# jstrom2002/ImageCodecs

Measured on NVIDIA B200. Metric: jpeg_encode_mp_per_s, higher is better.
Workload: dtype f32

## Files before the change

### imagecodecs_b200/csrc/jpeg_tables.h

```cpp
#pragma once
#include <stddef.h>
#include <stdint.h>

namespace jg {

#define JG_ZZ_INIT                                                                              \
    { 0, 1, 5, 6, 14, 15, 27, 28, 2, 4, 7, 13, 16, 26, 29, 42, 3, 8, 12, 17, 25, 30, 41, 43,    \
      9, 11, 18, 24, 31, 40, 44, 53, 10, 19, 23, 32, 39, 45, 52, 54, 20, 22, 33, 38, 46, 51,    \
      55, 60, 21, 34, 37, 47, 50, 56, 59, 61, 35, 36, 48, 49, 57, 58, 62, 63 }

enum HuffTable { HT_LUMA_DC = 0, HT_LUMA_AC = 1, HT_CHROMA_DC = 2, HT_CHROMA_AC = 3 };

enum Layout { LAYOUT_444 = 0, LAYOUT_420 = 1, LAYOUT_GRAY = 2 };

struct QuantSet {
    float luma[64];
    float chroma[64];
};

struct HuffLut {
    uint32_t ac[2][256];
    uint32_t dc[2][16];
};

bool build_qt(int quality_mode, int quality, uint8_t qt_luma[64], uint8_t qt_chroma[64]);
void build_pqt(const uint8_t qt[64], float pqt[64]);
void build_huff_lut(HuffLut* lut);
size_t emit_headers(int w, int h, int ncomp_out, int subsampling, const uint8_t qt_luma[64],
                    const uint8_t qt_chroma[64], uint8_t* out, size_t cap, int restart_interval = 0);
size_t schedule_words(int n_images);
size_t build_schedule(const int* tiles_per_image, int n_images, uint32_t* out);

}
```

### imagecodecs_b200/csrc/jpeg_transform.cuh

```cuda
#pragma once
#include "jpeg_kernel.cuh"

namespace jg {

template <int LAYOUT>
struct TGeo {
    static constexpr int BPM = LAYOUT == LAYOUT_444 ? 3 : (LAYOUT == LAYOUT_420 ? 6 : 1);
    static constexpr int ITER_MCUS = LAYOUT == LAYOUT_420 ? 2 : 8;
    static constexpr int ITERS = LAYOUT == LAYOUT_444 ? 4 : 8;
    static constexpr int ITEM_MCUS = ITER_MCUS * ITERS;
    static constexpr int ITER_BLOCKS = ITER_MCUS * BPM;
    static constexpr int GROUP_FLOATS = LAYOUT == LAYOUT_444 ? 3 * 2 * kTileFloats : (LAYOUT == LAYOUT_420 ? 6 * kTileFloats : 2 * kTileFloats);
    static constexpr int GROUPS = LAYOUT == LAYOUT_420 ? 2 : 4;
    static constexpr int MCU_PAD = LAYOUT == LAYOUT_420 ? 48 : (LAYOUT == LAYOUT_444 ? 24 : 0);
    static constexpr int STAGE_INT16 = ITER_BLOCKS * kCoefStride + ITER_MCUS * MCU_PAD;
    static JG_DEV int stage_off(int b) { return b * kCoefStride + (b / BPM) * MCU_PAD; }
    static JG_DEV int stage_off(int mcu, int j) { return (mcu * BPM + j) * kCoefStride + mcu * MCU_PAD; }
};
static_assert(TGeo<LAYOUT_444>::ITEM_MCUS == transform_item_mcus(LAYOUT_444) && TGeo<LAYOUT_420>::ITEM_MCUS == transform_item_mcus(LAYOUT_420) &&
              TGeo<LAYOUT_GRAY>::ITEM_MCUS == transform_item_mcus(LAYOUT_GRAY), "host and kernel agree on the item size");

template <int LAYOUT>
struct TWarp {
    using G = TGeo<LAYOUT>;
    alignas(16) float xch[G::GROUPS * G::GROUP_FLOATS];
    alignas(16) int16_t stage[G::STAGE_INT16];
};
template <int LAYOUT>
struct TSmem { TWarp<LAYOUT> wm[kWarps]; };

struct TLane {
    float pq_l[8], pq_c[8];
    unsigned zz2[8];
};

constexpr float kFloorMagic = 12582912.0f - 1024.0f;
JG_DEV void quantise2(f32x2 c, float pq, unsigned& kx, unsigned& ky)
{
    const f32x2 b = f2_add(f2_add(f2_mul(c, f2(pq, pq)), f2(1024.0f, 1024.0f)), f2(0.5f, 0.5f));
    const f32x2 r = f2_add_rd(b, f2(kFloorMagic, kFloorMagic));
    kx = f_bits(r.x);
    ky = f_bits(r.y);
}
JG_DEV unsigned quantise1(float c, float pq)
{
    return f_bits(f_add_rd(f_add(f_add(f_mul(c, pq), 1024.0f), 0.5f), kFloorMagic));
}
template <int NC>
JG_DEV void rgb_biased(const uint32_t* w, int i, float& r, float& g, float& b)
{
    if (NC == 4) { r = u8_biased(w[i], 0); g = u8_biased(w[i], 1); b = u8_biased(w[i], 2); }
    else {
        r = u8_biased(w[(3 * i) >> 2], (3 * i) & 3);
        g = u8_biased(w[(3 * i + 1) >> 2], (3 * i + 1) & 3);
        b = u8_biased(w[(3 * i + 2) >> 2], (3 * i + 2) & 3);
    }
}
#ifndef JG_U8_VIA_PRMT
#define JG_U8_VIA_PRMT 1
#endif
template <int NC>
JG_DEV void rgb_pair(const uint32_t* wa, const uint32_t* wb, int ia, int ib, f32x2& R, f32x2& G, f32x2& B)
{
    float r0, g0, b0, r1, g1, b1;
#if JG_U8_VIA_PRMT
    rgb_biased<NC>(wa, ia, r0, g0, b0);
    rgb_biased<NC>(wb, ib, r1, g1, b1);
    const f32x2 bias = f2(kU8Bias, kU8Bias);
    R = f2_sub(f2(r0, r1), bias); G = f2_sub(f2(g0, g1), bias); B = f2_sub(f2(b0, b1), bias);
#else
    rgb_of<NC>(wa, ia, r0, g0, b0);
    rgb_of<NC>(wb, ib, r1, g1, b1);
    R = f2(r0, r1); G = f2(g0, g1); B = f2(b0, b1);
#endif
}

struct TAddr {
    unsigned xch;
    unsigned stage;
};

template <int LAYOUT>
JG_DEV void stage_to_global(unsigned stage, int16_t* gout, int nblk)
{
    using G = TGeo<LAYOUT>;
    const int t = JG_TID & 31;
#pragma unroll
    for (int q = 0; q < (G::ITER_BLOCKS * 8 + 31) / 32; ++q) {
        const int c = q * 32 + t, blk = c >> 3, part = c & 7;
        if (blk < nblk) *reinterpret_cast<uint4*>(gout + blk * 64 + part * 8) = lds_v4(stage + (unsigned)(G::stage_off(blk) + part * 8) * 2u);
    }
}

template <int LAYOUT, int NC>
struct TPixels {
    static constexpr int WORDS = LAYOUT == LAYOUT_420 ? 16 * NC / 4 : (LAYOUT == LAYOUT_444 ? 8 * NC / 4 : 2);
    uint32_t a[WORDS];
    uint32_t b[LAYOUT == LAYOUT_420 ? 1 : WORDS];
};

template <int LAYOUT, int NC>
JG_DEV void fetch_pixels(const ImageDesc& im, int my0, int mx0, int nM, TPixels<LAYOUT, NC>& px)
{
    const int t = JG_TID & 31, u = t & 7;
#pragma unroll
    for (int i = 0; i < TPixels<LAYOUT, NC>::WORDS; ++i) px.a[i] = 0u;
    if (LAYOUT == LAYOUT_420) {
        const int grp = t >> 4, r16 = t & 15;
        if (grp < nM) {
            int my, mx;
            mcu_pos(im, my0, mx0, grp, my, mx);
            int y = my * 16 + r16; if (y >= im.h) y = im.h - 1;
            load_segment<NC, 16>(im, mx * 16, y, reinterpret_cast<uint32_t (&)[16 * NC / 4]>(px.a));
        }
    } else {
        constexpr int C = LAYOUT == LAYOUT_444 ? NC : 1;
        const int g = t >> 3;
        const int sa = LAYOUT == LAYOUT_444 ? g : 2 * g, sb = LAYOUT == LAYOUT_444 ? g + 4 : 2 * g + 1;
#pragma unroll
        for (int i = 0; i < TPixels<LAYOUT, NC>::WORDS; ++i) px.b[i] = 0u;
        if (sa < nM) {
            int my, mx;
            mcu_pos(im, my0, mx0, sa, my, mx);
            int y = my * 8 + u; if (y >= im.h) y = im.h - 1;
            load_segment<C, 8>(im, mx * 8, y, reinterpret_cast<uint32_t (&)[8 * C / 4]>(px.a));
        }
        if (sb < nM) {
            int my, mx;
            mcu_pos(im, my0, mx0, sb, my, mx);
            int y = my * 8 + u; if (y >= im.h) y = im.h - 1;
            load_segment<C, 8>(im, mx * 8, y, reinterpret_cast<uint32_t (&)[8 * C / 4]>(px.b));
        }
    }
}

template <int NC, class Prefetch>
JG_DEV void transform_iter_444(const TAddr& A, const TPixels<LAYOUT_444, NC>& px, int nM, int16_t* gout, const TLane& LC, Prefetch&& prefetch)
{
    const int t = JG_TID & 31, u = t & 7, g = t >> 3;
    f32x2 sy[8], sb[8], sr[8];
#pragma unroll
    for (int i = 0; i < 8; ++i) {
        f32x2 R, Gc, B;
        rgb_pair<NC>(px.a, px.b, i, i, R, Gc, B);
        sy[i] = f2_sub(f2_add(f2_add(f2_mul(f2(0.299f, 0.299f), R), f2_mul(f2(0.587f, 0.587f), Gc)), f2_mul(f2(0.114f, 0.114f), B)),
                       f2(128.0f, 128.0f));
        sb[i] = f2_add(f2_sub(f2_mul(f2(-0.1687f, -0.1687f), R), f2_mul(f2(0.3313f, 0.3313f), Gc)), f2_mul(f2(0.5f, 0.5f), B));
        sr[i] = f2_sub(f2_sub(f2_mul(f2(0.5f, 0.5f), R), f2_mul(f2(0.4187f, 0.4187f), Gc)), f2_mul(f2(0.0813f, 0.0813f), B));
    }
    prefetch();
    const unsigned row = A.xch + (unsigned)(u * 9) * 8u;
    aan8x2(sy);
#pragma unroll
    for (int i = 0; i < 8; ++i) sts_v2f(row + 8u * i, sy[i]);
    aan8x2(sb);
#pragma unroll
    for (int i = 0; i < 8; ++i) sts_v2f(row + 8u * (kTileFloats + i), sb[i]);
    aan8x2(sr);
#pragma unroll
    for (int i = 0; i < 8; ++i) sts_v2f(row + 8u * (2 * kTileFloats + i), sr[i]);
    warp_sync();
    const unsigned colA = A.xch + 8u * (unsigned)u;
#pragma unroll
    for (int c = 0; c < 3; ++c) {
        f32x2 col[8];
#pragma unroll
        for (int v = 0; v < 8; ++v) col[v] = lds_v2f(colA + 8u * (unsigned)(c * kTileFloats + v * 9));
        aan8x2(col);
        const unsigned dA = A.stage + 2u * (unsigned)TGeo<LAYOUT_444>::stage_off(g, c), dB = A.stage + 2u * (unsigned)TGeo<LAYOUT_444>::stage_off(g + 4, c);
#pragma unroll
        for (int v = 0; v < 8; ++v) {
            unsigned ka, kb;
            quantise2(col[v], c ? LC.pq_c[v] : LC.pq_l[v], ka, kb);
            sts_u16(dA + LC.zz2[v], ka);
            sts_u16(dB + LC.zz2[v], kb);
        }
    }
    warp_sync();
    stage_to_global<LAYOUT_444>(A.stage, gout, nM * 3);
}

template <int NC, class Prefetch>
JG_DEV void transform_iter_420(const TAddr& A, const TPixels<LAYOUT_420, NC>& px, int nM, int16_t* gout, const TLane& LC, Prefetch&& prefetch)
{
    const int t = JG_TID & 31, u = t & 7, grp = t >> 4, r16 = t & 15, h = r16 >> 3;
    const unsigned ypair = A.xch;
    const unsigned ctile = A.xch + 4u * (4 * kTileFloats);
    const bool valid = grp < nM;
    f32x2 cbs[4], crs[4];
    f32x2 sy[8];
#pragma unroll
    for (int j = 0; j < 4; ++j) {
        f32x2 cb[2], cr[2];
#pragma unroll
        for (int e = 0; e < 2; ++e) {
            const int i = 2 * j + e;
            f32x2 R, Gc, B;
            rgb_pair<NC>(px.a, px.a, i, i + 8, R, Gc, B);
            sy[i] = f2_sub(f2_add(f2_add(f2_mul(f2(0.299f, 0.299f), R), f2_mul(f2(0.587f, 0.587f), Gc)),
                                  f2_mul(f2(0.114f, 0.114f), B)), f2(128.0f, 128.0f));
            cb[e] = f2_add(f2_sub(f2_mul(f2(-0.1687f, -0.1687f), R), f2_mul(f2(0.3313f, 0.3313f), Gc)),
                           f2_mul(f2(0.5f, 0.5f), B));
            cr[e] = f2_sub(f2_sub(f2_mul(f2(0.5f, 0.5f), R), f2_mul(f2(0.4187f, 0.4187f), Gc)),
                           f2_mul(f2(0.0813f, 0.0813f), B));
        }
        cbs[j] = f2_add(cb[0], cb[1]);
        crs[j] = f2_add(cr[0], cr[1]);
    }
    prefetch();
    aan8x2(sy);
    if (valid) {
        const unsigned ty = ypair + 8u * (unsigned)(h * kTileFloats + (r16 & 7) * 9);
#pragma unroll
        for (int i = 0; i < 8; ++i) sts_v2f(ty + 8u * i, sy[i]);
    }
    const bool even = (r16 & 1) == 0;
    float samp[8];
#pragma unroll
    for (int i = 0; i < 4; ++i) {
        const f32x2 mine = even ? cbs[i] : crs[i], give = even ? crs[i] : cbs[i];
        const f32x2 other = f2(warp_shfl_xor_f32(give.x, 1), warp_shfl_xor_f32(give.y, 1));
        const f32x2 q = f2_mul(f2_add(mine, other), f2(0.25f, 0.25f));
        samp[i] = q.x; samp[4 + i] = q.y;
    }
    aan8(samp);
    if (valid) {
        const unsigned tc = ctile + 4u * (unsigned)((r16 & 1) * kTileFloats + (r16 >> 1) * 9);
#pragma unroll
        for (int i = 0; i < 8; ++i) sts_f32(tc + 4u * i, samp[i]);
    }
    warp_sync();
    if (valid) {
        f32x2 col[8];
#pragma unroll
        for (int v = 0; v < 8; ++v) col[v] = lds_v2f(ypair + 8u * (unsigned)(h * kTileFloats + v * 9 + u));
        aan8x2(col);
        const unsigned dL = A.stage + 2u * (unsigned)TGeo<LAYOUT_420>::stage_off(grp, 2 * h), dR = dL + 2u * kCoefStride;
#pragma unroll
        for (int v = 0; v < 8; ++v) {
            unsigned kl, kr;
            quantise2(col[v], LC.pq_l[v], kl, kr);
            sts_u16(dL + LC.zz2[v], kl);
            sts_u16(dR + LC.zz2[v], kr);
        }
        float c[8];
#pragma unroll
        for (int v = 0; v < 8; ++v) c[v] = lds_f32(ctile + 4u * (unsigned)(h * kTileFloats + v * 9 + u));
        aan8(c);
        const unsigned dC = A.stage + 2u * (unsigned)TGeo<LAYOUT_420>::stage_off(grp, 4 + h);
#pragma unroll
        for (int v = 0; v < 8; ++v) sts_u16(dC + LC.zz2[v], quantise1(c[v], LC.pq_c[v]));
    }
    warp_sync();
    stage_to_global<LAYOUT_420>(A.stage, gout, nM * 6);
}

template <class Prefetch>
JG_DEV void transform_iter_gray(const TAddr& A, const TPixels<LAYOUT_GRAY, 1>& px, int nM, int16_t* gout, const TLane& LC, Prefetch&& prefetch)
{
    const int t = JG_TID & 31, u = t & 7, g = t >> 3;
    f32x2 s[8];
#if JG_U8_VIA_PRMT
#pragma unroll
    for (int i = 0; i < 8; ++i)
        s[i] = f2_sub(f2_sub(f2(u8_biased(px.a[i >> 2], i & 3), u8_biased(px.b[i >> 2], i & 3)), f2(kU8Bias, kU8Bias)), f2(128.0f, 128.0f));
#else
#pragma unroll
    for (int i = 0; i < 8; ++i) s[i] = f2_sub(f2(u8_to_f(byte_of(px.a, i)), u8_to_f(byte_of(px.b, i))), f2(128.0f, 128.0f));
#endif
    prefetch();
    aan8x2(s);
#pragma unroll
    for (int i = 0; i < 8; ++i) sts_v2f(A.xch + 8u * (unsigned)(u * 9 + i), s[i]);
    warp_sync();
    f32x2 col[8];
#pragma unroll
    for (int v = 0; v < 8; ++v) col[v] = lds_v2f(A.xch + 8u * (unsigned)(v * 9 + u));
    aan8x2(col);
    const unsigned dA = A.stage + 2u * (unsigned)((2 * g) * kCoefStride), dB = dA + 2u * kCoefStride;
#pragma unroll
    for (int v = 0; v < 8; ++v) {
        unsigned ka, kb;
        quantise2(col[v], LC.pq_l[v], ka, kb);
        sts_u16(dA + LC.zz2[v], ka);
        sts_u16(dB + LC.zz2[v], kb);
    }
    warp_sync();
    stage_to_global<LAYOUT_GRAY>(A.stage, gout, nM);
}

#ifndef JG_TR_MINB
#define JG_TR_MINB (LAYOUT == LAYOUT_444 ? 3 : 4)
#endif
template <int LAYOUT, int NC>
JG_KERNEL(kThreads, JG_TR_MINB)
void transform_kernel(const JG_GRID_CONSTANT TransformParams P, const JG_GRID_CONSTANT QuantSet Q)
{
    using G = TGeo<LAYOUT>;
    JG_DYNAMIC_SMEM(smem_raw);
    TSmem<LAYOUT>& S = *reinterpret_cast<TSmem<LAYOUT>*>(smem_raw);
    const int t = JG_TID;
    const unsigned item = (unsigned)JG_CTA_ID * (unsigned)kWarps + (unsigned)(t >> 5);
    if (item >= (unsigned)P.n_items) return;
    TLane LC;
    {
        const int u = t & 7;
#pragma unroll
        for (int v = 0; v < 8; ++v) {
            LC.pq_l[v] = Q.luma[8 * v + u];
            LC.pq_c[v] = Q.chroma[8 * v + u];
            LC.zz2[v] = 2u * (unsigned)zz_of(8 * v + u);
        }
    }
    unsigned img, local;
    if (P.items_per_image > 0) {
        img = item / (unsigned)P.items_per_image;
        local = item - img * (unsigned)P.items_per_image;
    } else {
        unsigned lo = 0, hi = (unsigned)P.n_images - 1u;
        while (lo < hi) {
            const unsigned mid = (lo + hi + 1u) >> 1;
            if (ldg_u32(P.first_item + mid) <= item) lo = mid; else hi = mid - 1u;
        }
        img = lo;
        local = item - ldg_u32(P.first_item + lo);
    }
    const ImageDesc im = P.images[img];
    TWarp<LAYOUT>& W = S.wm[t >> 5];
    TAddr A;
    A.xch = smem_addr(W.xch) + 4u * (unsigned)(((t & 31) / (32 / G::GROUPS)) * G::GROUP_FLOATS);
    A.stage = smem_addr(W.stage);
    const int m_begin = (int)local * G::ITEM_MCUS;
    const int m_end = (im.n_mcus - m_begin < G::ITEM_MCUS) ? im.n_mcus : m_begin + G::ITEM_MCUS;
    int16_t* gout = P.coefs + (im.first_block + (unsigned long long)m_begin * G::BPM) * 64ull;
    int my0 = m_begin / im.mcus_x, mx0 = m_begin - my0 * im.mcus_x;
    TPixels<LAYOUT, NC> px;
    fetch_pixels<LAYOUT, NC>(im, my0, mx0, m_end - m_begin < G::ITER_MCUS ? m_end - m_begin : G::ITER_MCUS, px);
#pragma unroll 1
    for (int m0 = m_begin; m0 < m_end; m0 += G::ITER_MCUS) {
        const int nM = m_end - m0 < G::ITER_MCUS ? m_end - m0 : G::ITER_MCUS;
        int mx1 = mx0 + G::ITER_MCUS, my1 = my0;
        while (mx1 >= im.mcus_x) { mx1 -= im.mcus_x; ++my1; }
        const int left = m_end - m0 - G::ITER_MCUS;
        const int nM1 = left < 0 ? 0 : (left < G::ITER_MCUS ? left : G::ITER_MCUS);
        TPixels<LAYOUT, NC> nx;
        auto prefetch = [&]() { fetch_pixels<LAYOUT, NC>(im, my1, mx1, nM1, nx); };
        if constexpr (LAYOUT == LAYOUT_444) transform_iter_444<NC>(A, px, nM, gout, LC, prefetch);
        else if constexpr (LAYOUT == LAYOUT_420) transform_iter_420<NC>(A, px, nM, gout, LC, prefetch);
        else transform_iter_gray(A, px, nM, gout, LC, prefetch);
        px = nx;
        gout += G::ITER_BLOCKS * 64;
        mx0 = mx1; my0 = my1;
    }
}

}
```

### imagecodecs_b200/csrc/jpeg_device.h

```cpp
#pragma once
#include <stdint.h>

#if defined(JG_EMULATE)
#include "cuda_emu.h"
#else
#include <cuda_runtime.h>

#define JG_DEV __device__ __forceinline__
#define JG_DEV_NOINLINE __device__ __noinline__
#define JG_TID ((int)threadIdx.x)
#define JG_CTA_ID ((int)blockIdx.x)
#define JG_GRID_DIM ((int)gridDim.x)
#define JG_KERNEL(threads, min_ctas) __global__ __launch_bounds__(threads, min_ctas)
#define JG_GRID_CONSTANT __grid_constant__
#define JG_DYNAMIC_SMEM(name) extern __shared__ __align__(16) unsigned char name[]
#define JG_CONST_TABLE static __device__ __constant__
#define JG_WARP_ANY(x) __any_sync(0xffffffffu, (x))
#define JG_RECONVERGE() __syncwarp()

namespace jg {

JG_DEV float f_add(float a, float b) { return __fadd_rn(a, b); }
JG_DEV float f_sub(float a, float b) { return __fsub_rn(a, b); }
JG_DEV float f_mul(float a, float b) { return __fmul_rn(a, b); }
// ... 95 lines not shown
JG_DEV void mbar_init(unsigned long long* bar, unsigned arrivals)
{
    asm volatile("mbarrier.init.shared::cta.b64 [%0], %1;" ::"r"(smem_addr(bar)), "r"(arrivals) : "memory");
}
JG_DEV void mbar_fence_init() { asm volatile("fence.mbarrier_init.release.cluster;" ::: "memory"); }
JG_DEV void mbar_expect_tx(unsigned long long* bar, unsigned bytes)
{
    asm volatile("mbarrier.arrive.expect_tx.shared::cta.b64 _, [%0], %1;" ::"r"(smem_addr(bar)), "r"(bytes) : "memory");
}
JG_DEV void bulk_g2s(void* dst_smem, const void* src_gmem, unsigned bytes, unsigned long long* bar)
{
    asm volatile("cp.async.bulk.shared::cluster.global.mbarrier::complete_tx::bytes [%0], [%1], %2, [%3];"
                 ::"r"(smem_addr(dst_smem)), "l"(src_gmem), "r"(bytes), "r"(smem_addr(bar)) : "memory");
}
JG_DEV void fence_proxy_async() { asm volatile("fence.proxy.async.shared::cta;" ::: "memory"); }
JG_DEV void tma_load_2d(void* dst_smem, const void* tmap, int c0, int c1, unsigned long long* bar)
{
    asm volatile("cp.async.bulk.tensor.2d.shared::cluster.global.tile.mbarrier::complete_tx::bytes [%0], [%1, {%2, %3}], [%4];"
                 ::"r"(smem_addr(dst_smem)), "l"(tmap), "r"(c0), "r"(c1), "r"(smem_addr(bar)) : "memory");
}
JG_DEV void mbar_wait(unsigned long long* bar, unsigned parity)
{
    asm volatile(
        "{\n"
        ".reg .pred p;\n"
        "WAIT_%=:\n"
        "mbarrier.try_wait.parity.shared::cta.b64 p, [%0], %1;\n"
        "@!p bra WAIT_%=;\n"
        "}\n" ::"r"(smem_addr(bar)), "r"(parity) : "memory");
}

}
#endif
```

### imagecodecs_b200/csrc/jpeg_entropy.cu

```cuda
#include "jpeg_entropy.cuh"
#include "jpeg_launch.h"

namespace jg {

template <int MODE>
static cudaError_t entropy_prepare_mode(int* ctas)
{
    auto kern = entropy_kernel<MODE>;
    const int smem = (int)sizeof(EntSmem);
    cudaError_t e = cudaFuncSetAttribute(kern, cudaFuncAttributeMaxDynamicSharedMemorySize, smem);
    if (e != cudaSuccess) return e;
    int n = 0;
    e = cudaOccupancyMaxActiveBlocksPerMultiprocessor(&n, kern, kEntThreads, smem);
    if (n < *ctas) *ctas = n;
    return e;
}

cudaError_t entropy_prepare(int* ctas_per_sm)
{
    int ctas = 1 << 20;
    cudaError_t e = entropy_prepare_mode<kEntModePlain>(&ctas);
    if (e == cudaSuccess) e = entropy_prepare_mode<kEntModeRestart>(&ctas);
    *ctas_per_sm = ctas;
    return e;
}

cudaError_t entropy_launch(int grid, cudaStream_t stream, const LaunchParams& P, const CoefMap& cmap, bool restart)
{
    const size_t smem = sizeof(EntSmem);
    if (restart) entropy_kernel<kEntModeRestart><<<grid, kEntThreads, smem, stream>>>(P, cmap);
    else entropy_kernel<kEntModePlain><<<grid, kEntThreads, smem, stream>>>(P, cmap);
    return cudaGetLastError();
}

}
```

### imagecodecs_b200/csrc/jpeg_entropy.cuh

```cuda
#pragma once
#include "jpeg_kernel.cuh"

namespace jg {

constexpr int kEntBlocks = 32;
constexpr int kEntCoefStride = 72;
#ifndef JG_ENT_SUBWORDS
#define JG_ENT_SUBWORDS 24
#endif
constexpr int kSubWords = JG_ENT_SUBWORDS;
constexpr int kEntRegionWords = 768;
#ifndef JG_ENT_PIECE
#define JG_ENT_PIECE 96
#endif
constexpr int kOnePieceSymbols = JG_ENT_PIECE * kSubWords;
constexpr int kSlowBlocks = 4;
constexpr int kEntModePlain = 0, kEntModeRestart = 2;
constexpr unsigned kEntStageBytes = kEntBlocks * kEntCoefStride * 2;
constexpr unsigned kTabRunBytes = 136u, kTabAcBytes = 16u * kTabRunBytes;
constexpr unsigned kTabDc = 0u, kTabAc = 2u, kTabChroma = 1u, kTabAcChroma = kTabAcBytes / 128u;
static_assert(kTabAcBytes % 128u == 0u, "table offsets are multiples of 128 bytes");

struct EntWarp {
    alignas(128) int16_t coef[kEntBlocks * kEntCoefStride];
// ... 333 lines not shown
        flush_region(W.region, tg, pd.last && hi == nblk, reinterpret_cast<uint8_t*>(pd.raw), pd.raw_cap, k, hb, pos, cap_overflow);
    }
    if (lane == 0) {
        if (pd.last) P.raw_bytes[pd.img_idx] = pos;
        if (cap_overflow) gmem_atomic_or(P.img_status + pd.img_idx, 1u);
    }
    warp_sync();
    clear_region(W.region, kEntRegionWords + 8);
    return true;
}

template <int MODE>
JG_KERNEL(kEntThreads, JG_ENT_MINB)
void entropy_kernel(const JG_GRID_CONSTANT LaunchParams P, const JG_GRID_CONSTANT CoefMap cmap)
{
    constexpr bool restart = MODE == kEntModeRestart;
    JG_DYNAMIC_SMEM(smem_raw);
    EntSmem& S = *reinterpret_cast<EntSmem*>(smem_raw);
    const int t = JG_TID, lane = t & 31;
    for (int i = t; i < 32 + 512; i += kEntThreads) {
        const int cls = i < 32 ? i >> 4 : (i - 32) >> 8, k = i < 32 ? i & 15 : (i - 32) & 255;
        const unsigned h = i < 32 ? P.huff->dc[cls][k] : P.huff->ac[cls][k];
        uint2 e;
        e.x = h >> 8;
        e.y = (h & 0xffu) + (unsigned)(k & 15);
        S.tab.e[i < 32 ? i : (256u + (unsigned)cls * kTabAcBytes) / 8u + (unsigned)(k >> 4) * 17u + (unsigned)(k & 15)] = e;
    }
    EntWarp& W = S.wm[t >> 5];
    const EntTables& T = S.tab;
    if (lane == 0) mbar_init(&W.mbar, 1u);
    clear_region(W.region, kEntRegionWords + 8);
    if (lane < 4) { uint2 z; z.x = 0u; z.y = 0u; W.rec[kEntBlocks + lane] = z; }
    mbar_fence_init();
    cta_sync();

    const int bpm = P.bpm, bpt = P.blocks_per_tile;
    const int lane_j = lane % bpm;
    unsigned phase = 0;
    PendingOut po;
    for (int slot = 0;; slot ^= 1) {
        int img_idx;
        const int g = draw_tile(P, img_idx);
        const bool have = g < P.n_tiles;
        int nblk = 0, b0 = 0, jb = 0, pred_outside = 0;
        bool first = false;
        if (have) {
            const ImageDesc im = P.images[img_idx];
            const int lt = g - im.first_tile;
            const int n_blocks = im.n_mcus * bpm;
            b0 = lt * bpt;
            nblk = n_blocks - b0 < bpt ? n_blocks - b0 : bpt;
            first = lt == 0;
            jb = b0 % bpm;
            if (lane == 0) {
                fence_proxy_async();
                mbar_expect_tx(&W.mbar, kEntStageBytes);
                tma_load_2d(W.coef, &cmap, 0, (int)(im.first_block + (unsigned long long)b0), &W.mbar);
            }
            if (!restart && lane < nblk) {
                int j = jb + lane_j; if (j >= bpm) j -= bpm;
                unsigned cls; int delta;
                block_role(bpm, j, cls, delta);
                const int ps = lane - delta;
                if (ps < 0 && b0 + ps >= 0)
                    pred_outside = (int)ldg_s16(P.coefs + (im.first_block + (unsigned long long)(b0 + ps)) * 64ull);
            }
// ... 51 lines not shown
```

### imagecodecs_b200/csrc/jpeg_launch.h

```cpp
#pragma once
#include <stddef.h>
#include <stdint.h>

#if !defined(JG_EMULATE)
#include <cuda_runtime.h>
#endif

#include "jpeg_tables.h"

namespace jg {

constexpr int kThreads = 128;
constexpr int kBlocksPerTile = 24;
constexpr int kWarps = kThreads / 32;
constexpr int kChunkBytes = 64 * kThreads;

constexpr int mcus_per_tile(int layout) { return layout == LAYOUT_444 ? 8 : (layout == LAYOUT_420 ? 4 : 24); }
constexpr int kWinWordsMax = 384;
constexpr int kWinWordsMin = 216;
constexpr unsigned kSpinLimit = 1u << 24;
#ifndef JG_DEEP_MAX_IMAGES
#define JG_DEEP_MAX_IMAGES 48
#endif
constexpr int kDeepMaxImages = JG_DEEP_MAX_IMAGES;
// ... 37 lines not shown
    unsigned long long* raw_bytes;
    unsigned* first_chunk;
    unsigned long long* scan_bytes;
    unsigned* img_status;
    const HuffLut* huff;
    int16_t* dbg_coefs;
    uint32_t* dbg_bits;
    const int16_t* coefs;
    int bpm;
    int blocks_per_tile;
};

constexpr int kEntTileBlocks = 32, kEntTileBlocksRestart = 24;
#ifndef JG_ENT_WARPS
#define JG_ENT_WARPS 20
#endif
#ifndef JG_ENT_MINB
#define JG_ENT_MINB 1
#endif
constexpr int kEntWarps = JG_ENT_WARPS, kEntThreads = 32 * kEntWarps;
struct alignas(64) CoefMap { unsigned long long q[16]; };

struct TransformParams {
    const ImageDesc* images;
    int n_images;
    int n_items;
    int items_per_image;
    const uint32_t* first_item;
    int16_t* coefs;
};
constexpr int transform_item_mcus(int layout) { return layout == LAYOUT_444 ? 32 : (layout == LAYOUT_420 ? 16 : 64); }

#if !defined(JG_EMULATE)
#define JG_DECLARE_SPEC(L, N)                                                                   \
    size_t smem_bytes_##L##_##N();                                                              \
    cudaError_t prepare_##L##_##N(int* ctas_per_sm);                                            \
    cudaError_t launch_##L##_##N(int grid, cudaStream_t stream, const LaunchParams& P, const QuantSet& Q, int mode);      \
    cudaError_t transform_prepare_##L##_##N();                                                                            \
    cudaError_t transform_launch_##L##_##N(cudaStream_t stream, const struct TransformParams& P, const QuantSet& Q);
JG_DECLARE_SPEC(0, 3)
JG_DECLARE_SPEC(0, 4)
JG_DECLARE_SPEC(1, 3)
JG_DECLARE_SPEC(1, 4)
JG_DECLARE_SPEC(2, 1)
#undef JG_DECLARE_SPEC
cudaError_t entropy_prepare(int* ctas_per_sm);
cudaError_t entropy_launch(int grid, cudaStream_t stream, const LaunchParams& P, const CoefMap& cmap, bool restart);
size_t stuff_smem_bytes();
cudaError_t stuff_prepare(int* ctas_per_sm);
cudaError_t stuff_launch(int grid, cudaStream_t stream, const LaunchParams& P);
#endif

}
```

### imagecodecs_b200/csrc/jpeg_stuff.cu

```cuda
#include "jpeg_stuff.cuh"

namespace jg {

size_t stuff_smem_bytes() { return sizeof(StuffSmem); }

cudaError_t stuff_prepare(int* ctas_per_sm)
{
    return cudaOccupancyMaxActiveBlocksPerMultiprocessor(ctas_per_sm, stuff_kernel, kThreads, sizeof(StuffSmem));
}

cudaError_t stuff_launch(int grid, cudaStream_t stream, const LaunchParams& P)
{
    plan_chunks_kernel<<<1, kThreads, sizeof(ScanSmem), stream>>>(P);
    cudaError_t e = cudaGetLastError();
    if (e != cudaSuccess) return e;
    count_ff_kernel<<<grid, kCountThreads, sizeof(CountSmem), stream>>>(P);
    if ((e = cudaGetLastError()) != cudaSuccess) return e;
    scan_groups_kernel<<<1, kThreads, sizeof(ScanSmem), stream>>>(P);
    if ((e = cudaGetLastError()) != cudaSuccess) return e;
    stuff_kernel<<<grid, kThreads, sizeof(StuffSmem), stream>>>(P);
    return cudaGetLastError();
}

}
```

### imagecodecs_b200/csrc/jpeg_stuff.cuh

```cuda
#pragma once
#include "jpeg_device.h"
#include "jpeg_kernel.cuh"
#include "jpeg_launch.h"

namespace jg {

constexpr int kMaxMarks = kChunkBytes / 12 + 2;

struct StuffSmem {
    alignas(16) uint8_t sbuf[2 * kChunkBytes + 2 * kMaxMarks + 64];
    uint32_t warp_tmp[kWarps];
    uint32_t mark[kMaxMarks + 1];
    unsigned warp_ff[kWarps];
    unsigned n_marks, first_mark;
};
constexpr int kGroupChunks = 32;
struct CountSmem { unsigned cnt[kGroupChunks]; int img[kGroupChunks]; };
struct ScanSmem { uint32_t warp_tmp[kWarps]; };

JG_DEV unsigned long long tile_end_byte(const LaunchParams& P, const ImageDesc& im, unsigned j)
{
    return (ld_flag64(P.desc_bits + im.first_tile + j) & kCountMask) >> 3;
}
JG_DEV unsigned tile_ends_below(const LaunchParams& P, const ImageDesc& im, unsigned n, unsigned long long x)
{
    unsigned lo = 0, hi = n;
    while (lo < hi) {
        const unsigned mid = (lo + hi) >> 1;
        if (tile_end_byte(P, im, mid) < x) lo = mid + 1; else hi = mid;
    }
    return lo;
}

JG_KERNEL(kThreads, 1)
void plan_chunks_kernel(const JG_GRID_CONSTANT LaunchParams P)
{
    JG_DYNAMIC_SMEM(smem_raw);
    ScanSmem& S = *reinterpret_cast<ScanSmem*>(smem_raw);
    const int t = JG_TID;
    unsigned carry = 0;
    for (int i0 = 0; i0 < P.n_images; i0 += kThreads) {
        const int i = i0 + t;
        unsigned n = 0;
        if (i < P.n_images) {
            const unsigned long long rb = P.raw_bytes[i];
            if (P.img_status[i] & 1u) P.scan_bytes[i] = 2ull * rb + 2ull;
            else n = (unsigned)((rb + kChunkBytes - 1) / kChunkBytes);
        }
        unsigned tot;
        const unsigned ex = cta_scan_excl(n, S.warp_tmp, tot);
        if (i < P.n_images) P.first_chunk[i] = carry + ex;
        carry += tot;
    }
    if (t == 0) P.first_chunk[P.n_images] = carry;
}

JG_DEV int image_of_chunk(const LaunchParams& P, unsigned c, int lane)
{
    int lo = 0, hi = P.n_images - 1;
    while (lo < hi) {
        const int step = (hi - lo) / 32 + 1;
        const int probe = lo + (lane + 1) * step;
        const int ok = probe <= hi && P.first_chunk[probe <= hi ? probe : hi] <= c;
        const int k = i_popc(warp_ballot(ok));
        lo += k * step;
        if (lo + step - 1 < hi) hi = lo + step - 1;
    }
    return lo;
}
// ... 3 lines not shown
    const uint8_t* src = im.raw + off;
    unsigned cnt = 0;
    constexpr int NV = kChunkBytes / 512;
#pragma unroll 8
    for (int k = 0; k < NV; ++k) {
        const unsigned b = (unsigned)(k * 32 + lane) * 16u;
        if (b < nb) {
            uint4 v = ldg_u128(src + b);
            if (nb - b < 16u) {
                const unsigned v4 = nb - b;
                unsigned* w = &v.x;
#pragma unroll
                for (int j = 0; j < 4; ++j) {
                    const int have = (int)v4 - 4 * j;
                    if (have <= 0) w[j] = 0u; else if (have < 4) w[j] &= 0xffffffffu >> (8 * (4 - have));
                }
            }
            cnt += (unsigned)(i_popc(v_cmpeq4(v.x, 0xffffffffu)) + i_popc(v_cmpeq4(v.y, 0xffffffffu)) +
                              i_popc(v_cmpeq4(v.z, 0xffffffffu)) + i_popc(v_cmpeq4(v.w, 0xffffffffu)));
        }
    }
    unsigned total = warp_sum_u32(cnt >> 3);
    if ((im.flags & kFlagRestart) != 0 && im.n_tiles > 1) {
        const unsigned n_ends = (unsigned)im.n_tiles - 1u;
        total += 2u * (tile_ends_below(P, im, n_ends, off + nb) - tile_ends_below(P, im, n_ends, off));
    }
    return total;
}

constexpr int kCountThreads = 32 * kGroupChunks;
JG_KERNEL(kCountThreads, 2)
void count_ff_kernel(const JG_GRID_CONSTANT LaunchParams P)
{
    JG_DYNAMIC_SMEM(smem_raw);
    CountSmem& S = *reinterpret_cast<CountSmem*>(smem_raw);
    const int t = JG_TID, lane = t & 31, wq = t >> 5;
    const unsigned n_chunks = P.first_chunk[P.n_images];
    const unsigned n_groups = (n_chunks + kGroupChunks - 1) / kGroupChunks;
    for (unsigned g = (unsigned)JG_CTA_ID; g < n_groups; g += (unsigned)JG_GRID_DIM) {
        const unsigned c = g * kGroupChunks + (unsigned)wq;
        unsigned extra = 0;
        int img = 0;
        if (c < n_chunks) {
            img = image_of_chunk(P, c, lane);
            const ImageDesc im = P.images[img];
            const unsigned long long raw_n = P.raw_bytes[img];
            const unsigned long long off = (unsigned long long)(c - P.first_chunk[img]) * kChunkBytes;
            const unsigned nb = raw_n - off < (unsigned long long)kChunkBytes ? (unsigned)(raw_n - off) : (unsigned)kChunkBytes;
            extra = count_extra_bytes(P, im, off, nb, lane);
        }
        if (lane == 0) { S.cnt[wq] = extra; S.img[wq] = img; }
        cta_sync();
        if (wq == 0) {
            const unsigned v = S.cnt[lane];
            const unsigned inc = warp_scan_incl_u32(v);
            const unsigned cl = g * kGroupChunks + (unsigned)lane;
            if (cl < n_chunks) P.desc_ff[cl] = ((unsigned long long)(unsigned)S.img[lane] << 32) | (unsigned long long)(inc - v);
            if (lane == 31) P.ff_groups[g] = inc;
        }
        cta_sync();
    }
}

JG_KERNEL(kThreads, 1)
void scan_groups_kernel(const JG_GRID_CONSTANT LaunchParams P)
{
    JG_DYNAMIC_SMEM(smem_raw);
    ScanSmem& S = *reinterpret_cast<ScanSmem*>(smem_raw);
    const int t = JG_TID;
    const unsigned n_chunks = P.first_chunk[P.n_images];
    const unsigned n_groups = (n_chunks + kGroupChunks - 1) / kGroupChunks;
    const unsigned per = (n_groups + kThreads - 1) / kThreads;
    const unsigned lo = (unsigned)t * per, hi = lo + per < n_groups ? lo + per : n_groups;
    unsigned sum = 0;
    for (unsigned i = lo; i < hi; ++i) sum += P.ff_groups[i];
    unsigned tot;
    unsigned run = cta_scan_excl(sum, S.warp_tmp, tot);
    for (unsigned i = lo; i < hi; ++i) { const unsigned v = P.ff_groups[i]; P.ff_groups[i] = run; run += v; }
}

JG_DEV unsigned extra_before(const LaunchParams& P, unsigned c, unsigned long long d)
{
    return P.ff_groups[c / kGroupChunks] + (unsigned)d;
}

JG_DEV unsigned stuff_plain_chunk(const LaunchParams& P, StuffSmem& S, const ImageDesc& im, int img, unsigned ff_base,
                              unsigned long long off, unsigned nb, bool last_chunk, int t)
{
    constexpr int ROWS = kChunkBytes / (kWarps * 128);
    const int lane = t & 31, wq = t >> 5;
    const unsigned wbase = (unsigned)wq * (ROWS * 128u) + 4u * (unsigned)lane;
    const uint8_t* src = im.raw + off + wbase;
    unsigned w[ROWS];
#pragma unroll
    for (int q = 0; q < ROWS; ++q) w[q] = wbase + 128u * q < nb ? ldg_u32(src + 128 * q) : 0u;
    if (nb < (unsigned)kChunkBytes) {
#pragma unroll
        for (int q = 0; q < ROWS; ++q) {
            const int v = (int)nb - (int)(wbase + 128u * q);
// ... 131 lines not shown
        if (head > out_bytes) head = out_bytes;
        const unsigned nvec = (out_bytes - head) >> 4;
        const unsigned tail0 = head + (nvec << 4);
        const uint32_t* sw = reinterpret_cast<const uint32_t*>(S.sbuf);
        if ((unsigned)t < head) dst[t] = S.sbuf[t];
        uint4* dst4 = reinterpret_cast<uint4*>(dst + head);
        for (unsigned i = (unsigned)t; i < nvec; i += kThreads) {
            const unsigned o = head + (i << 4);
            const unsigned wi = o >> 2, sh = (o & 3u) * 8u;
            uint4 r;
            if (sh == 0) { r.x = sw[wi]; r.y = sw[wi + 1]; r.z = sw[wi + 2]; r.w = sw[wi + 3]; }
            else {
                const unsigned a0 = sw[wi], a1 = sw[wi + 1], a2 = sw[wi + 2], a3 = sw[wi + 3], a4 = sw[wi + 4];
                r.x = (a0 >> sh) | (a1 << (32u - sh)); r.y = (a1 >> sh) | (a2 << (32u - sh));
                r.z = (a2 >> sh) | (a3 << (32u - sh)); r.w = (a3 >> sh) | (a4 << (32u - sh));
            }
            dst4[i] = r;
        }
        if (tail0 + (unsigned)t < out_bytes) dst[tail0 + t] = S.sbuf[tail0 + t];
    }
    if (t == 0) {
        if (!fits) gmem_atomic_or(P.img_status + img, 1u);
        if (last_chunk) {
            if (fits) { im.out[pos + out_bytes] = 0xFF; im.out[pos + out_bytes + 1] = 0xD9; }
            P.scan_bytes[img] = pos + out_bytes + 2;
        }
    }
    return ff_chunk;
}

JG_KERNEL(kThreads, 8)
void stuff_kernel(const JG_GRID_CONSTANT LaunchParams P)
{
    JG_DYNAMIC_SMEM(smem_raw);
    StuffSmem& S = *reinterpret_cast<StuffSmem*>(smem_raw);
    const int t = JG_TID;
    const unsigned n_chunks = P.first_chunk[P.n_images];
    if (ld_flag32(P.error) != 0u) return;
    const unsigned per = (n_chunks + (unsigned)JG_GRID_DIM - 1u) / (unsigned)JG_GRID_DIM;
    const unsigned c_begin = (unsigned)JG_CTA_ID * per, c_end = c_begin + per < n_chunks ? c_begin + per : n_chunks;
    int img = 0;
    unsigned first = 0, next_first = 0, ff_base = 0;
    unsigned long long raw_n = 0;
    ImageDesc im;
    for (unsigned c = c_begin; c < c_end; ++c) {
        if (c == c_begin || c >= next_first) {
            const unsigned long long d = P.desc_ff[c];
            img = (int)(d >> 32);
            first = P.first_chunk[img];
            next_first = P.first_chunk[img + 1];
            im = P.images[img];
            raw_n = P.raw_bytes[img];
            ff_base = extra_before(P, c, d) - extra_before(P, first, P.desc_ff[first]);
        }
        const unsigned long long off = (unsigned long long)(c - first) * kChunkBytes;
        const unsigned nb = raw_n - off < (unsigned long long)kChunkBytes ? (unsigned)(raw_n - off) : (unsigned)kChunkBytes;
        const bool last_chunk = off + nb == raw_n;
        if ((im.flags & kFlagRestart) != 0 && im.n_tiles > 1) ff_base += stuff_restart_chunk(P, S, im, img, ff_base, off, nb, last_chunk, t);
        else ff_base += stuff_plain_chunk(P, S, im, img, ff_base, off, nb, last_chunk, t);
        cta_sync();
    }
}

}
```

Baseline: 240,300.

## Store quantised columns vectorised and apply zigzag in registers at batched flush

For the 4:4:4 and 4:2:0 layouts, each lane now packs its eight quantised coefficients into one 16-byte shared store in column order, replacing eight scattered 16-bit zigzag stores. Several iterations are staged together, up to 32 blocks. At flush time each lane takes one block, reorders it into zigzag order with byte permutes generated at compile time, writes it back, and the warp then copies the whole group to global memory. This is meant to cut shared-memory store instructions and bank conflicts and to batch global writes. In exchange the stage buffer grows, the per-MCU padding is dropped, the flush adds a full-block register pass (64 registers per lane), and lanes sit idle while a partial group is flushed.

Result: faster. 244,300 (median of 6 runs) (+1.7%).

```diff
diff --git a/imagecodecs_b200/csrc/jpeg_tables.h b/imagecodecs_b200/csrc/jpeg_tables.h
--- a/imagecodecs_b200/csrc/jpeg_tables.h
+++ b/imagecodecs_b200/csrc/jpeg_tables.h
@@ -8,6 +8,15 @@
     { 0, 1, 5, 6, 14, 15, 27, 28, 2, 4, 7, 13, 16, 26, 29, 42, 3, 8, 12, 17, 25, 30, 41, 43,    \
       9, 11, 18, 24, 31, 40, 44, 53, 10, 19, 23, 32, 39, 45, 52, 54, 20, 22, 33, 38, 46, 51,    \
       55, 60, 21, 34, 37, 47, 50, 56, 59, 61, 35, 36, 48, 49, 57, 58, 62, 63 }
+
+constexpr int col_of_zz(int k)
+{
+    constexpr unsigned char zz[64] = JG_ZZ_INIT;
+    int n = 0;
+    while (zz[n] != k) ++n;
+    return 8 * (n & 7) + (n >> 3);
+}
+static_assert(col_of_zz(0) == 0 && col_of_zz(1) == 8 && col_of_zz(2) == 1 && col_of_zz(63) == 63, "column order keeps the DC and (7, 7) in place");
 
 enum HuffTable { HT_LUMA_DC = 0, HT_LUMA_AC = 1, HT_CHROMA_DC = 2, HT_CHROMA_AC = 3 };
 
diff --git a/imagecodecs_b200/csrc/jpeg_transform.cuh b/imagecodecs_b200/csrc/jpeg_transform.cuh
--- a/imagecodecs_b200/csrc/jpeg_transform.cuh
+++ b/imagecodecs_b200/csrc/jpeg_transform.cuh
@@ -12,11 +12,13 @@
     static constexpr int ITER_BLOCKS = ITER_MCUS * BPM;
     static constexpr int GROUP_FLOATS = LAYOUT == LAYOUT_444 ? 3 * 2 * kTileFloats : (LAYOUT == LAYOUT_420 ? 6 * kTileFloats : 2 * kTileFloats);
     static constexpr int GROUPS = LAYOUT == LAYOUT_420 ? 2 : 4;
-    static constexpr int MCU_PAD = LAYOUT == LAYOUT_420 ? 48 : (LAYOUT == LAYOUT_444 ? 24 : 0);
-    static constexpr int STAGE_INT16 = ITER_BLOCKS * kCoefStride + ITER_MCUS * MCU_PAD;
-    static JG_DEV int stage_off(int b) { return b * kCoefStride + (b / BPM) * MCU_PAD; }
-    static JG_DEV int stage_off(int mcu, int j) { return (mcu * BPM + j) * kCoefStride + mcu * MCU_PAD; }
-};
+    static constexpr int FLUSH_ITERS = LAYOUT == LAYOUT_GRAY ? 1 : 32 / ITER_BLOCKS;
+    static constexpr int FLUSH_BLOCKS = FLUSH_ITERS * ITER_BLOCKS;
+    static constexpr int STAGE_INT16 = FLUSH_BLOCKS * kCoefStride;
+    static_assert(LAYOUT != LAYOUT_GRAY || FLUSH_BLOCKS == 8, "gray stages one iteration");
+};
+static_assert(TGeo<LAYOUT_444>::ITERS % TGeo<LAYOUT_444>::FLUSH_ITERS == 0 && TGeo<LAYOUT_420>::ITERS % TGeo<LAYOUT_420>::FLUSH_ITERS == 0 &&
+              TGeo<LAYOUT_GRAY>::ITERS % TGeo<LAYOUT_GRAY>::FLUSH_ITERS == 0, "an item is whole reorder groups");
 static_assert(TGeo<LAYOUT_444>::ITEM_MCUS == transform_item_mcus(LAYOUT_444) && TGeo<LAYOUT_420>::ITEM_MCUS == transform_item_mcus(LAYOUT_420) &&
               TGeo<LAYOUT_GRAY>::ITEM_MCUS == transform_item_mcus(LAYOUT_GRAY), "host and kernel agree on the item size");
 
@@ -75,20 +77,52 @@
 #endif
 }
 
-struct TAddr {
-    unsigned xch;
-    unsigned stage;
-};
+JG_DEV void store_column(int16_t* blk, int u, const unsigned (&k)[8])
+{
+    uint4 w;
+    w.x = byte_perm(k[0], k[1], 0x5410u);
+    w.y = byte_perm(k[2], k[3], 0x5410u);
+    w.z = byte_perm(k[4], k[5], 0x5410u);
+    w.w = byte_perm(k[6], k[7], 0x5410u);
+    *reinterpret_cast<uint4*>(blk + 8 * u) = w;
+}
+
+template <int W>
+struct ZzWord {
+    static constexpr int a = col_of_zz(2 * W), b = col_of_zz(2 * W + 1);
+    static constexpr unsigned sel = (a & 1 ? 0x32u : 0x10u) | (b & 1 ? 0x7600u : 0x5400u);
+};
+template <int W = 0>
+JG_DEV void to_zigzag(const unsigned (&c)[32], unsigned (&z)[32])
+{
+    z[W] = byte_perm(c[ZzWord<W>::a >> 1], c[ZzWord<W>::b >> 1], ZzWord<W>::sel);
+    if constexpr (W < 31) to_zigzag<W + 1>(c, z);
+}
 
 template <int LAYOUT>
-JG_DEV void stage_to_global(unsigned stage, int16_t* gout, int nblk)
+JG_DEV void zigzag_to_global(TWarp<LAYOUT>& W, int16_t* gout, int nblk)
 {
     using G = TGeo<LAYOUT>;
     const int t = JG_TID & 31;
-#pragma unroll
-    for (int q = 0; q < (G::ITER_BLOCKS * 8 + 31) / 32; ++q) {
+    const unsigned stage = smem_addr(W.stage);
+    if (LAYOUT != LAYOUT_GRAY && t < nblk) {
+        const unsigned a = stage + 2u * (unsigned)(t * kCoefStride);
+        unsigned c[32], z[32];
+#pragma unroll
+        for (int q = 0; q < 8; ++q) {
+            const uint4 v = lds_v4(a + 16u * (unsigned)q);
+            c[4 * q] = v.x; c[4 * q + 1] = v.y; c[4 * q + 2] = v.z; c[4 * q + 3] = v.w;
+        }
+        to_zigzag(c, z);
+        uint4* row = reinterpret_cast<uint4*>(W.stage + t * kCoefStride);
+#pragma unroll
+        for (int q = 0; q < 8; ++q) { const uint4 v = {z[4 * q], z[4 * q + 1], z[4 * q + 2], z[4 * q + 3]}; row[q] = v; }
+    }
+    warp_sync();
+#pragma unroll
+    for (int q = 0; q < (G::FLUSH_BLOCKS * 8 + 31) / 32; ++q) {
         const int c = q * 32 + t, blk = c >> 3, part = c & 7;
-        if (blk < nblk) *reinterpret_cast<uint4*>(gout + blk * 64 + part * 8) = lds_v4(stage + (unsigned)(G::stage_off(blk) + part * 8) * 2u);
+        if (blk < nblk) *reinterpret_cast<uint4*>(gout + blk * 64 + part * 8) = lds_v4(stage + (unsigned)(blk * kCoefStride + part * 8) * 2u);
     }
 }
 
@@ -135,7 +169,7 @@
 }
 
 template <int NC, class Prefetch>
-JG_DEV void transform_iter_444(const TAddr& A, const TPixels<LAYOUT_444, NC>& px, int nM, int16_t* gout, const TLane& LC, Prefetch&& prefetch)
+JG_DEV void transform_iter_444(unsigned xch, int16_t* stg, const TPixels<LAYOUT_444, NC>& px, int nM, const TLane& LC, Prefetch&& prefetch)
 {
     const int t = JG_TID & 31, u = t & 7, g = t >> 3;
     f32x2 sy[8], sb[8], sr[8];
@@ -149,7 +183,7 @@
         sr[i] = f2_sub(f2_sub(f2_mul(f2(0.5f, 0.5f), R), f2_mul(f2(0.4187f, 0.4187f), Gc)), f2_mul(f2(0.0813f, 0.0813f), B));
     }
     prefetch();
-    const unsigned row = A.xch + (unsigned)(u * 9) * 8u;
+    const unsigned row = xch + (unsigned)(u * 9) * 8u;
     aan8x2(sy);
 #pragma unroll
     for (int i = 0; i < 8; ++i) sts_v2f(row + 8u * i, sy[i]);
@@ -160,32 +194,28 @@
 #pragma unroll
     for (int i = 0; i < 8; ++i) sts_v2f(row + 8u * (2 * kTileFloats + i), sr[i]);
     warp_sync();
-    const unsigned colA = A.xch + 8u * (unsigned)u;
+    const unsigned colA = xch + 8u * (unsigned)u;
 #pragma unroll
     for (int c = 0; c < 3; ++c) {
         f32x2 col[8];
 #pragma unroll
         for (int v = 0; v < 8; ++v) col[v] = lds_v2f(colA + 8u * (unsigned)(c * kTileFloats + v * 9));
         aan8x2(col);
-        const unsigned dA = A.stage + 2u * (unsigned)TGeo<LAYOUT_444>::stage_off(g, c), dB = A.stage + 2u * (unsigned)TGeo<LAYOUT_444>::stage_off(g + 4, c);
-#pragma unroll
-        for (int v = 0; v < 8; ++v) {
-            unsigned ka, kb;
-            quantise2(col[v], c ? LC.pq_c[v] : LC.pq_l[v], ka, kb);
-            sts_u16(dA + LC.zz2[v], ka);
-            sts_u16(dB + LC.zz2[v], kb);
-        }
-    }
-    warp_sync();
-    stage_to_global<LAYOUT_444>(A.stage, gout, nM * 3);
+        unsigned ka[8], kb[8];
+#pragma unroll
+        for (int v = 0; v < 8; ++v) quantise2(col[v], c ? LC.pq_c[v] : LC.pq_l[v], ka[v], kb[v]);
+        store_column(stg + (g * 3 + c) * kCoefStride, u, ka);
+        store_column(stg + ((g + 4) * 3 + c) * kCoefStride, u, kb);
+    }
+    warp_sync();
 }
 
 template <int NC, class Prefetch>
-JG_DEV void transform_iter_420(const TAddr& A, const TPixels<LAYOUT_420, NC>& px, int nM, int16_t* gout, const TLane& LC, Prefetch&& prefetch)
+JG_DEV void transform_iter_420(unsigned xch, int16_t* stg, const TPixels<LAYOUT_420, NC>& px, int nM, const TLane& LC, Prefetch&& prefetch)
 {
     const int t = JG_TID & 31, u = t & 7, grp = t >> 4, r16 = t & 15, h = r16 >> 3;
-    const unsigned ypair = A.xch;
-    const unsigned ctile = A.xch + 4u * (4 * kTileFloats);
+    const unsigned ypair = xch;
+    const unsigned ctile = xch + 4u * (4 * kTileFloats);
     const bool valid = grp < nM;
     f32x2 cbs[4], crs[4];
     f32x2 sy[8];
@@ -235,28 +265,26 @@
 #pragma unroll
         for (int v = 0; v < 8; ++v) col[v] = lds_v2f(ypair + 8u * (unsigned)(h * kTileFloats + v * 9 + u));
         aan8x2(col);
-        const unsigned dL = A.stage + 2u * (unsigned)TGeo<LAYOUT_420>::stage_off(grp, 2 * h), dR = dL + 2u * kCoefStride;
-#pragma unroll
-        for (int v = 0; v < 8; ++v) {
-            unsigned kl, kr;
-            quantise2(col[v], LC.pq_l[v], kl, kr);
-            sts_u16(dL + LC.zz2[v], kl);
-            sts_u16(dR + LC.zz2[v], kr);
-        }
+        int16_t* mcu = stg + grp * (6 * kCoefStride);
+        unsigned kl[8], kr[8];
+#pragma unroll
+        for (int v = 0; v < 8; ++v) quantise2(col[v], LC.pq_l[v], kl[v], kr[v]);
+        store_column(mcu + (2 * h) * kCoefStride, u, kl);
+        store_column(mcu + (2 * h + 1) * kCoefStride, u, kr);
         float c[8];
 #pragma unroll
         for (int v = 0; v < 8; ++v) c[v] = lds_f32(ctile + 4u * (unsigned)(h * kTileFloats + v * 9 + u));
         aan8(c);
-        const unsigned dC = A.stage + 2u * (unsigned)TGeo<LAYOUT_420>::stage_off(grp, 4 + h);
-#pragma unroll
-        for (int v = 0; v < 8; ++v) sts_u16(dC + LC.zz2[v], quantise1(c[v], LC.pq_c[v]));
-    }
-    warp_sync();
-    stage_to_global<LAYOUT_420>(A.stage, gout, nM * 6);
+        unsigned kc[8];
+#pragma unroll
+        for (int v = 0; v < 8; ++v) kc[v] = quantise1(c[v], LC.pq_c[v]);
+        store_column(mcu + (4 + h) * kCoefStride, u, kc);
+    }
+    warp_sync();
 }
 
 template <class Prefetch>
-JG_DEV void transform_iter_gray(const TAddr& A, const TPixels<LAYOUT_GRAY, 1>& px, int nM, int16_t* gout, const TLane& LC, Prefetch&& prefetch)
+JG_DEV void transform_iter_gray(unsigned xch, int16_t* stg, const TPixels<LAYOUT_GRAY, 1>& px, int nM, const TLane& LC, Prefetch&& prefetch)
 {
     const int t = JG_TID & 31, u = t & 7, g = t >> 3;
     f32x2 s[8];
@@ -271,13 +299,13 @@
     prefetch();
     aan8x2(s);
 #pragma unroll
-    for (int i = 0; i < 8; ++i) sts_v2f(A.xch + 8u * (unsigned)(u * 9 + i), s[i]);
+    for (int i = 0; i < 8; ++i) sts_v2f(xch + 8u * (unsigned)(u * 9 + i), s[i]);
     warp_sync();
     f32x2 col[8];
 #pragma unroll
-    for (int v = 0; v < 8; ++v) col[v] = lds_v2f(A.xch + 8u * (unsigned)(v * 9 + u));
+    for (int v = 0; v < 8; ++v) col[v] = lds_v2f(xch + 8u * (unsigned)(v * 9 + u));
     aan8x2(col);
-    const unsigned dA = A.stage + 2u * (unsigned)((2 * g) * kCoefStride), dB = dA + 2u * kCoefStride;
+    const unsigned dA = smem_addr(stg + (2 * g) * kCoefStride), dB = dA + 2u * kCoefStride;
 #pragma unroll
     for (int v = 0; v < 8; ++v) {
         unsigned ka, kb;
@@ -286,7 +314,6 @@
         sts_u16(dB + LC.zz2[v], kb);
     }
     warp_sync();
-    stage_to_global<LAYOUT_GRAY>(A.stage, gout, nM);
 }
 
 #ifndef JG_TR_MINB
@@ -309,7 +336,7 @@
         for (int v = 0; v < 8; ++v) {
             LC.pq_l[v] = Q.luma[8 * v + u];
             LC.pq_c[v] = Q.chroma[8 * v + u];
-            LC.zz2[v] = 2u * (unsigned)zz_of(8 * v + u);
+            if (LAYOUT == LAYOUT_GRAY) LC.zz2[v] = 2u * (unsigned)zz_of(8 * v + u);
         }
     }
     unsigned img, local;
@@ -327,15 +354,14 @@
     }
     const ImageDesc im = P.images[img];
     TWarp<LAYOUT>& W = S.wm[t >> 5];
-    TAddr A;
-    A.xch = smem_addr(W.xch) + 4u * (unsigned)(((t & 31) / (32 / G::GROUPS)) * G::GROUP_FLOATS);
-    A.stage = smem_addr(W.stage);
+    const unsigned xch = smem_addr(W.xch) + 4u * (unsigned)(((t & 31) / (32 / G::GROUPS)) * G::GROUP_FLOATS);
     const int m_begin = (int)local * G::ITEM_MCUS;
     const int m_end = (im.n_mcus - m_begin < G::ITEM_MCUS) ? im.n_mcus : m_begin + G::ITEM_MCUS;
     int16_t* gout = P.coefs + (im.first_block + (unsigned long long)m_begin * G::BPM) * 64ull;
     int my0 = m_begin / im.mcus_x, mx0 = m_begin - my0 * im.mcus_x;
     TPixels<LAYOUT, NC> px;
     fetch_pixels<LAYOUT, NC>(im, my0, mx0, m_end - m_begin < G::ITER_MCUS ? m_end - m_begin : G::ITER_MCUS, px);
+    int slot = 0;
 #pragma unroll 1
     for (int m0 = m_begin; m0 < m_end; m0 += G::ITER_MCUS) {
         const int nM = m_end - m0 < G::ITER_MCUS ? m_end - m0 : G::ITER_MCUS;
@@ -345,11 +371,18 @@
         const int nM1 = left < 0 ? 0 : (left < G::ITER_MCUS ? left : G::ITER_MCUS);
         TPixels<LAYOUT, NC> nx;
         auto prefetch = [&]() { fetch_pixels<LAYOUT, NC>(im, my1, mx1, nM1, nx); };
-        if constexpr (LAYOUT == LAYOUT_444) transform_iter_444<NC>(A, px, nM, gout, LC, prefetch);
-        else if constexpr (LAYOUT == LAYOUT_420) transform_iter_420<NC>(A, px, nM, gout, LC, prefetch);
-        else transform_iter_gray(A, px, nM, gout, LC, prefetch);
+        int16_t* stg = W.stage + slot * (G::ITER_BLOCKS * kCoefStride);
+        if constexpr (LAYOUT == LAYOUT_444) transform_iter_444<NC>(xch, stg, px, nM, LC, prefetch);
+        else if constexpr (LAYOUT == LAYOUT_420) transform_iter_420<NC>(xch, stg, px, nM, LC, prefetch);
+        else transform_iter_gray(xch, stg, px, nM, LC, prefetch);
+        if (slot == G::FLUSH_ITERS - 1 || m0 + G::ITER_MCUS >= m_end) {
+            zigzag_to_global<LAYOUT>(W, gout, slot * G::ITER_BLOCKS + nM * G::BPM);
+            gout += G::FLUSH_BLOCKS * 64;
+            slot = 0;
+        } else {
+            ++slot;
+        }
         px = nx;
-        gout += G::ITER_BLOCKS * 64;
         mx0 = mx1; my0 = my1;
     }
 }
```

## Use programmatic dependent launch to overlap kernel launches in the encode pipeline

Applied to the files above, without the earlier changes.

Launches the entropy, chunk-planning, FF-counting, group-scan and stuffing kernels with the programmatic stream serialization attribute. Each dependent kernel calls griddepcontrol.wait before touching upstream data, and every kernel triggers dependents early. This lets the launch latency and prologue of the next kernel overlap the tail of the previous one in a chain of small kernels. The risk is extra resident CTAs competing for SM resources while the prior grid is still running.

Measured after the change: 240,300 before, 241,400 after (median of 6 runs). About the same (+0.4%).

```diff
diff --git a/imagecodecs_b200/csrc/jpeg_device.h b/imagecodecs_b200/csrc/jpeg_device.h
--- a/imagecodecs_b200/csrc/jpeg_device.h
+++ b/imagecodecs_b200/csrc/jpeg_device.h
@@ -151,3 +151,13 @@
 
 }
 #endif
+
+namespace jg {
+#if defined(JG_EMULATE)
+inline void grid_dep_wait() {}
+inline void grid_dep_trigger() {}
+#else
+JG_DEV void grid_dep_wait() { asm volatile("griddepcontrol.wait;" ::: "memory"); }
+JG_DEV void grid_dep_trigger() { asm volatile("griddepcontrol.launch_dependents;" ::: "memory"); }
+#endif
+}
diff --git a/imagecodecs_b200/csrc/jpeg_entropy.cu b/imagecodecs_b200/csrc/jpeg_entropy.cu
--- a/imagecodecs_b200/csrc/jpeg_entropy.cu
+++ b/imagecodecs_b200/csrc/jpeg_entropy.cu
@@ -28,9 +28,8 @@
 cudaError_t entropy_launch(int grid, cudaStream_t stream, const LaunchParams& P, const CoefMap& cmap, bool restart)
 {
     const size_t smem = sizeof(EntSmem);
-    if (restart) entropy_kernel<kEntModeRestart><<<grid, kEntThreads, smem, stream>>>(P, cmap);
-    else entropy_kernel<kEntModePlain><<<grid, kEntThreads, smem, stream>>>(P, cmap);
-    return cudaGetLastError();
+    if (restart) return launch_dependent(entropy_kernel<kEntModeRestart>, grid, kEntThreads, smem, stream, P, cmap);
+    return launch_dependent(entropy_kernel<kEntModePlain>, grid, kEntThreads, smem, stream, P, cmap);
 }
 
 }
diff --git a/imagecodecs_b200/csrc/jpeg_entropy.cuh b/imagecodecs_b200/csrc/jpeg_entropy.cuh
--- a/imagecodecs_b200/csrc/jpeg_entropy.cuh
+++ b/imagecodecs_b200/csrc/jpeg_entropy.cuh
@@ -389,6 +389,8 @@
     clear_region(W.region, kEntRegionWords + 8);
     if (lane < 4) { uint2 z; z.x = 0u; z.y = 0u; W.rec[kEntBlocks + lane] = z; }
     mbar_fence_init();
+    grid_dep_wait();
+    grid_dep_trigger();
     cta_sync();
 
     const int bpm = P.bpm, bpt = P.blocks_per_tile;
diff --git a/imagecodecs_b200/csrc/jpeg_launch.h b/imagecodecs_b200/csrc/jpeg_launch.h
--- a/imagecodecs_b200/csrc/jpeg_launch.h
+++ b/imagecodecs_b200/csrc/jpeg_launch.h
@@ -93,6 +93,22 @@
 constexpr int transform_item_mcus(int layout) { return layout == LAYOUT_444 ? 32 : (layout == LAYOUT_420 ? 16 : 64); }
 
 #if !defined(JG_EMULATE)
+template <typename... Params, typename... Args>
+inline cudaError_t launch_dependent(void (*kern)(Params...), int grid, int threads, size_t smem, cudaStream_t stream, Args&&... args)
+{
+    cudaLaunchAttribute attr;
+    attr.id = cudaLaunchAttributeProgrammaticStreamSerialization;
+    attr.val.programmaticStreamSerializationAllowed = 1;
+    cudaLaunchConfig_t cfg = {};
+    cfg.gridDim = dim3((unsigned)grid);
+    cfg.blockDim = dim3((unsigned)threads);
+    cfg.dynamicSmemBytes = smem;
+    cfg.stream = stream;
+    cfg.attrs = &attr;
+    cfg.numAttrs = 1;
+    return cudaLaunchKernelEx(&cfg, kern, static_cast<Args&&>(args)...);
+}
+
 #define JG_DECLARE_SPEC(L, N)                                                                   \
     size_t smem_bytes_##L##_##N();                                                              \
     cudaError_t prepare_##L##_##N(int* ctas_per_sm);                                            \
diff --git a/imagecodecs_b200/csrc/jpeg_stuff.cu b/imagecodecs_b200/csrc/jpeg_stuff.cu
--- a/imagecodecs_b200/csrc/jpeg_stuff.cu
+++ b/imagecodecs_b200/csrc/jpeg_stuff.cu
@@ -11,15 +11,13 @@
 
 cudaError_t stuff_launch(int grid, cudaStream_t stream, const LaunchParams& P)
 {
-    plan_chunks_kernel<<<1, kThreads, sizeof(ScanSmem), stream>>>(P);
-    cudaError_t e = cudaGetLastError();
+    cudaError_t e = launch_dependent(plan_chunks_kernel, 1, kThreads, sizeof(ScanSmem), stream, P);
     if (e != cudaSuccess) return e;
-    count_ff_kernel<<<grid, kCountThreads, sizeof(CountSmem), stream>>>(P);
-    if ((e = cudaGetLastError()) != cudaSuccess) return e;
-    scan_groups_kernel<<<1, kThreads, sizeof(ScanSmem), stream>>>(P);
-    if ((e = cudaGetLastError()) != cudaSuccess) return e;
-    stuff_kernel<<<grid, kThreads, sizeof(StuffSmem), stream>>>(P);
-    return cudaGetLastError();
+    e = launch_dependent(count_ff_kernel, grid, kCountThreads, sizeof(CountSmem), stream, P);
+    if (e != cudaSuccess) return e;
+    e = launch_dependent(scan_groups_kernel, 1, kThreads, sizeof(ScanSmem), stream, P);
+    if (e != cudaSuccess) return e;
+    return launch_dependent(stuff_kernel, grid, kThreads, sizeof(StuffSmem), stream, P);
 }
 
 }
diff --git a/imagecodecs_b200/csrc/jpeg_stuff.cuh b/imagecodecs_b200/csrc/jpeg_stuff.cuh
--- a/imagecodecs_b200/csrc/jpeg_stuff.cuh
+++ b/imagecodecs_b200/csrc/jpeg_stuff.cuh
@@ -35,6 +35,8 @@
 JG_KERNEL(kThreads, 1)
 void plan_chunks_kernel(const JG_GRID_CONSTANT LaunchParams P)
 {
+    grid_dep_wait();
+    grid_dep_trigger();
     JG_DYNAMIC_SMEM(smem_raw);
     ScanSmem& S = *reinterpret_cast<ScanSmem*>(smem_raw);
     const int t = JG_TID;
@@ -104,6 +106,8 @@
 JG_KERNEL(kCountThreads, 2)
 void count_ff_kernel(const JG_GRID_CONSTANT LaunchParams P)
 {
+    grid_dep_wait();
+    grid_dep_trigger();
     JG_DYNAMIC_SMEM(smem_raw);
     CountSmem& S = *reinterpret_cast<CountSmem*>(smem_raw);
     const int t = JG_TID, lane = t & 31, wq = t >> 5;
@@ -137,6 +141,8 @@
 JG_KERNEL(kThreads, 1)
 void scan_groups_kernel(const JG_GRID_CONSTANT LaunchParams P)
 {
+    grid_dep_wait();
+    grid_dep_trigger();
     JG_DYNAMIC_SMEM(smem_raw);
     ScanSmem& S = *reinterpret_cast<ScanSmem*>(smem_raw);
     const int t = JG_TID;
@@ -334,6 +340,8 @@
 JG_KERNEL(kThreads, 8)
 void stuff_kernel(const JG_GRID_CONSTANT LaunchParams P)
 {
+    grid_dep_wait();
+    grid_dep_trigger();
     JG_DYNAMIC_SMEM(smem_raw);
     StuffSmem& S = *reinterpret_cast<StuffSmem*>(smem_raw);
     const int t = JG_TID;
diff --git a/imagecodecs_b200/csrc/jpeg_transform.cuh b/imagecodecs_b200/csrc/jpeg_transform.cuh
--- a/imagecodecs_b200/csrc/jpeg_transform.cuh
+++ b/imagecodecs_b200/csrc/jpeg_transform.cuh
@@ -300,6 +300,7 @@
     JG_DYNAMIC_SMEM(smem_raw);
     TSmem<LAYOUT>& S = *reinterpret_cast<TSmem<LAYOUT>*>(smem_raw);
     const int t = JG_TID;
+    grid_dep_trigger();
     const unsigned item = (unsigned)JG_CTA_ID * (unsigned)kWarps + (unsigned)(t >> 5);
     if (item >= (unsigned)P.n_items) return;
     TLane LC;
```
